# saamiya225/Graph-and-sequential-recommendation-systems

Measured on AMD Instinct MI355X. Metric: BPR training steps/sec (one step = K-layer LightGCN propagation + BPR loss + backward + Adam on a global batch of 2048 triplets), higher is better.
Workload: dtype bf16 (activation storage; f32 accumulation, parameters, gradients and Adam); 1 GPU; gowalla: 29858 users x 40981 items, 810128 train interactions, nnz(A_hat)=1620256, layers=3, dim=64, bpr_batch=2048; global_batch=2048, per_gpu_batch=2048, scaling_mode=strong, multi_gpu_status=n/a, parallelism=single GPU, act_dtype=bf16, xcd_remap=1, row_order=xcd

## Files before the change

graph-and-sequential-recommendation-systems_amd/_lib.py:

```python
import ctypes as C
import os

from . import build as _build

F32, BF16, FP8 = 0, 1, 2
ABI_VERSION = 13
MAX_LAYERS = 8

_c_i32p = C.POINTER(C.c_int32)
_c_i64p = C.POINTER(C.c_int64)
_c_f32p = C.POINTER(C.c_float)
_vp = C.c_void_p


def fp8_col_of_byte(d):
    import numpy as np
    b = np.arange(d)
    l, j, e = b // 16, (b % 16) // 4, b % 4
    return ((j * (d // 16) + l) * 4 + e).astype(np.int64)


class TrainConfig(C.Structure):
    _fields_ = [
        ("graph", _vp),
# ... 89 lines not shown
    "lgcn_train_step_cols_part2": (C.c_int, [_vp, _vp, _vp, _vp, C.c_int32, _vp, _vp]),
    "lgcn_dp_allreduce_sum_f32": (C.c_int, [_vp, _vp, C.c_int64, _vp]),
    "lgcn_dp_init_loopback": (C.c_int, [C.c_int, C.POINTER(_vp)]),
    "lgcn_dp_destroy": (None, [_vp]),
    "lgcn_dp_world": (C.c_int, [_vp]),
    "lgcn_dp_rank": (C.c_int, [_vp]),
    "lgcn_train_epoch_dp": (C.c_int, [_vp, _vp, _vp, _vp, _vp, C.c_int64, C.c_int32, C.c_int32, _vp, _vp, _vp, _vp]),
    "lgcn_rs_phase": (C.c_int, [_vp, C.c_int32, C.c_int32, _vp, _vp, _vp, C.c_int32, C.c_int32, C.c_int32, _vp, _vp, _vp]),
    "lgcn_rs_buffer": (C.c_int, [_vp, C.c_int32, C.c_int32, C.POINTER(_vp), C.POINTER(C.c_int32)]),
    "lgcn_ctx_set_dropout": (C.c_int, [_vp, C.c_float, C.c_uint64]),
    "lgcn_ctx_set_layer_weights": (C.c_int, [_vp, _vp, C.c_int32]),
    "lgcn_ctx_get_layer_weights": (C.c_int32, [_vp, _vp]),
    "lgcn_propagate_weighted": (C.c_int, [_vp, _vp, C.c_int, C.c_int, C.c_int, _vp, _vp, _vp, _vp]),
    "lgcn_dropout_mask": (C.c_int, [_vp, _vp, C.c_int64, C.c_int64, C.c_float, C.c_uint64, C.c_int64, _vp, _vp]),
    "lgcn_spmm_csr_drop": (C.c_int, [_vp, _vp, C.c_int, _vp, C.c_int, C.c_int, C.c_float, C.c_uint64, C.c_int64, C.c_int, _vp]),
    "lgcn_mf_create": (C.c_int, [C.POINTER(MfConfig), C.POINTER(_vp)]),
    "lgcn_mf_destroy": (None, [_vp]),
    "lgcn_mf_get_step": (C.c_int64, [_vp]),
    "lgcn_mf_set_step": (None, [_vp, C.c_int64]),
    "lgcn_mf_set_lr": (None, [_vp, C.c_double]),
    "lgcn_mf_train_step": (C.c_int, [_vp, _vp, _vp, _vp, C.c_int32, _vp, _vp]),
    "lgcn_mf_train_epoch": (C.c_int, [_vp, _vp, _vp, _vp, C.c_int64, C.c_int32, _vp, _vp]),
    "lgcn_mf_check": (C.c_int, [_vp, _vp]),
}

_LIB = None


class LgcnError(RuntimeError):
    pass


def load():
    global _LIB
    if _LIB is not None:
        return _LIB
    path = _build.LIB_PATH
    if os.environ.get("LGCN_LIB_PATH"):
        pass
    elif _build.is_stale():
        if _build.must_not_build():
            if not os.path.exists(path):
                raise LgcnError(
                    f"liblgcn_hip.so is missing at {path}; this process is a distributed rank or runs under a "
                    "profiler and will not compile it. Build it first (__graft_entry__.build()).")
        elif _build.find_hipcc() is not None:
# ... 380 lines not shown
```

graph-and-sequential-recommendation-systems_amd/csrc/lgcn_device.hip:

```cpp
#include <hip/hip_runtime.h>
#include <stdint.h>
#include <stdio.h>
#include <stdlib.h>
#include <string.h>
#include <math.h>
#include <algorithm>
#include <array>
#include <new>
#include <vector>

#include "lgcn_hip.h"
#include "lgcn_internal.h"

#define HIP_OK(expr)                                                            \
    do {                                                                        \
        hipError_t e_ = (expr);                                                 \
        if (e_ != hipSuccess) {                                                 \
            char buf_[256];                                                     \
            snprintf(buf_, sizeof buf_, "%s failed: %s", #expr, hipGetErrorString(e_)); \
            lgcn_set_error(buf_);                                               \
            return 10;                                                          \
        }                                                                       \
    } while (0)

// ... 848 lines not shown
    const float *X0; const void *Xl[LGCN_MAX_LAYERS + 1]; int K;
    int32_t n_users; int64_t N;
    const int32_t *users; const int32_t *pos; const int32_t *neg;
    int32_t B_local;
    int32_t shard;
    float inv_B;
    float lam;
    long long *G64;
    uint32_t *bitmap;
    uint32_t *stale_bitmap; int64_t bitmap_words;
    uint32_t *item_bitmap;
    float *contrib;
    int32_t exchange;
    const float *Xhub; int32_t hub_nnz;
    float *terms;
    int32_t terms_off, terms_stride;
    int32_t *err;
    int32_t dense_last;
    int32_t reg_ego;
    int32_t *cnt;
    int32_t cols_phase; float *erows; float *colsum;
    DropArgs dr;
    float w[LGCN_MAX_LAYERS + 1];
};

__device__ __forceinline__ float logsigmoid_f(float x) { return fminf(x, 0.f) - log1pf(expf(-fabsf(x))); }
__device__ __forceinline__ float sigmoid_neg_f(float x) {
    const float z = expf(-fabsf(x));
    return x < 0.f ? 1.f / (1.f + z) : z / (1.f + z);
}

__device__ __forceinline__ bool triplet_bad(const BprArgs &a, int b) {
    const int u = a.users[b], p = a.pos[b], n = a.neg[b];
    return u < 0 || u >= a.n_users || p < 0 || (int64_t)p + a.n_users >= a.N || n < 0 || (int64_t)n + a.n_users >= a.N;
}

template <int D>
__device__ __forceinline__ void triplet_finish(const BprArgs &a, int b, int l, const float *u, const float *p, const float *n,
                                               float ps, float ns, float rr);
template <int D>
__device__ __forceinline__ void triplet_loss_regs(const BprArgs &a, int b, int l, const float *u, const float *p, const float *n,
                                                  const float *u0 = nullptr, const float *p0 = nullptr, const float *n0 = nullptr) {
    constexpr int LPT = D < 64 ? D : 64, CPL = D / LPT;
    float ps = 0.f, ns = 0.f, ru = 0.f, rp = 0.f, rn = 0.f;
    const bool ego = a.reg_ego != 0;
    const float lam = ego ? 0.f : a.lam;
#pragma unroll
    for (int j = 0; j < CPL; j++) {
        ps += u[j] * p[j]; ns += u[j] * n[j];
        const float ur = ego ? u0[j] : u[j], pr = ego ? p0[j] : p[j], nr = ego ? n0[j] : n[j];
        ru += ur * ur; rp += pr * pr; rn += nr * nr;
    }
    float rr = ru + rp + rn;
#pragma unroll
    for (int off = 1; off < LPT; off <<= 1) {
        ps += __shfl_xor(ps, off); ns += __shfl_xor(ns, off); rr += __shfl_xor(rr, off);
    }
    if (a.cols_phase == 1) {
        const bool bad1 = triplet_bad(a, b);
        if (l == 0) { a.colsum[b] = bad1 ? 0.f : ps; a.colsum[a.B_local + b] = bad1 ? 0.f : ns; a.colsum[2 * a.B_local + b] = bad1 ? 0.f : rr; }
#pragma unroll
        for (int j = 0; j < CPL; j++) {
            a.erows[((int64_t)0 * a.B_local + b) * D + j * LPT + l] = u[j];
            a.erows[((int64_t)1 * a.B_local + b) * D + j * LPT + l] = p[j];
            a.erows[((int64_t)2 * a.B_local + b) * D + j * LPT + l] = n[j];
        }
        return;
    }
    triplet_finish<D>(a, b, l, u, p, n, ps, ns, rr);
}

template <int D>
__device__ __forceinline__ void triplet_finish(const BprArgs &a, int b, int l, const float *u, const float *p, const float *n,
                                               float ps, float ns, float rr) {
    constexpr int LPT = D < 64 ? D : 64, CPL = D / LPT;
    const float lam = a.reg_ego ? 0.f : a.lam;
    const bool tbad = triplet_bad(a, b);
    const float x = ps - ns;
    const float gb = tbad ? 0.f : -a.inv_B * sigmoid_neg_f(x);
    if (l == 0) {
        float *lt = a.exchange ? a.contrib + (int64_t)3 * a.shard * D : a.terms + a.terms_off;
        const int stride = a.exchange ? a.shard : a.terms_stride;
        lt[b] = tbad ? 0.f : logsigmoid_f(x);
        lt[stride + b] = tbad ? 0.f : rr;
    }
    if (tbad && !a.exchange) return;
    const int64_t rows[3] = {(int64_t)a.users[b], (int64_t)a.pos[b] + a.n_users, (int64_t)a.neg[b] + a.n_users};
#pragma unroll
    for (int c = 0; c < 3; c++) {
#pragma unroll
        for (int j = 0; j < CPL; j++) {
            float g = c == 0 ? gb * (p[j] - n[j]) + lam * u[j] : (c == 1 ? gb * u[j] + lam * p[j] : (-gb) * u[j] + lam * n[j]);
            if (a.G64 && !tbad)
                atomicAdd((unsigned long long *)(a.G64 + rows[c] * D + j * LPT + l),
                          (unsigned long long)__double2ll_rn((double)g * FIXED_SCALE));
            if (a.exchange) a.contrib[((int64_t)c * a.shard + b) * D + j * LPT + l] = tbad ? 0.f : g;
        }
        if (a.G64 && !tbad && l == 0) {
            atomicOr(a.bitmap + (rows[c] >> 5), 1u << (rows[c] & 31));
            if (a.cnt) atomicAdd(a.cnt + rows[c], 1);
            if (a.item_bitmap && c > 0) { const int64_t it = rows[c] - a.n_users; atomicOr(a.item_bitmap + (it >> 5), 1u << (it & 31)); }
        }
    }
}

#ifndef TRIPLET_HUB_NNZ
#define TRIPLET_HUB_NNZ 131072
#endif
#ifndef TRIPLET_HUB_CHUNK
#define TRIPLET_HUB_CHUNK 2048
#endif
#ifndef TRIPLET_MIN_WAVES
#define TRIPLET_MIN_WAVES 4
#endif
#ifndef TRIPLET_MIN_WAVES_F32
#define TRIPLET_MIN_WAVES_F32 7
#endif
#ifndef TRIPLET_U
#define TRIPLET_U LGCN_GATHER_U
#endif
#ifndef TRIPLET_WAVES
#define TRIPLET_WAVES 4
#endif
#ifndef TRIPLET_WAVES_BF16
#define TRIPLET_WAVES_BF16 3
#endif
// ... 469 lines not shown
    const int64_t blk = a.blk ? a.blk : (int64_t)3 * a.shard * D + 2 * a.shard;
    const float *src = a.gathered + r * blk + ((int64_t)c * a.shard + i) * D;
#pragma unroll
    for (int j = 0; j < CPT; j++)
        atomicAdd((unsigned long long *)(a.G64 + row * D + j * LPT + l),
                  (unsigned long long)__double2ll_rn((double)src[j * LPT + l] * FIXED_SCALE));
    if (l == 0) {
        atomicOr(a.bitmap + (row >> 5), 1u << (row & 31));
        if (a.cnt) atomicAdd(a.cnt + row, 1);
        if (a.item_bitmap && c > 0) { const int64_t it = row - a.n_users; atomicOr(a.item_bitmap + (it >> 5), 1u << (it & 31)); }
    }
}

template <int D>
__global__ void __launch_bounds__(256) k_g32(SlotArgs a) {
    constexpr int LPR = D / 4, SPB = 256 / LPR;
    const int s = blockIdx.x * SPB + threadIdx.x / LPR, l = threadIdx.x % LPR;
    if (s >= 3 * a.B) return;
    const int64_t row = slot_row(s / a.B, s % a.B, a.users, a.pos, a.neg, a.n_users, a.N);
    if (row < 0) return;
    store4(a.G32 + row * D + l * 4, loadv_fixed<4>(a.G64 + row * D + l * 4, a.div));
}

__global__ void __launch_bounds__(256) k_flag_rows(SlotArgs a) {
    const int s = blockIdx.x * 256 + threadIdx.x;
    if (s >= 3 * a.B) return;
    const int64_t row = slot_row(s / a.B, s % a.B, a.users, a.pos, a.neg, a.n_users, a.N);
    if (row >= 0) {
        atomicOr(a.bitmap + (row >> 5), 1u << (row & 31));
        if (a.cnt) atomicAdd(a.cnt + row, 1);
        if (a.item_bitmap && s >= a.B) { const int64_t it = row - a.n_users; atomicOr(a.item_bitmap + (it >> 5), 1u << (it & 31)); }
    }
}

template <int D>
__global__ void __launch_bounds__(256) k_finish(SlotArgs a) {
    constexpr int LPR = D / 4, SPB = 256 / LPR;
    const int s = blockIdx.x * SPB + threadIdx.x / LPR, l = threadIdx.x % LPR;
    if (s < 3 * a.B) {
        const int c = s / a.B, b = s % a.B;
        const int64_t row = slot_row(c, b, a.users, a.pos, a.neg, a.n_users, a.N);
        if (row >= 0) {
                    i64x2 *q = reinterpret_cast<i64x2 *>(a.G64 + row * D + l * 4);
            q[0] = i64x2{0, 0}; q[1] = i64x2{0, 0};
            if (l == 0) { a.bitmap[row >> 5] = 0u; if (a.cnt) a.cnt[row] = 0; }
        }
// ... 509 lines not shown
    int flip;
    void *act[LGCN_MAX_LAYERS + 1];
    int fwd_layers;
    float *g32;
    bf16_t *e0b;
    void *e0q;
    bool e0b_fresh;
    bool in_loop;
    lgcn_graph *hub_graph;
    int32_t hub_nnz;
    int64_t hub_rows;
    bool dp_local;
    int dp_rank;
    bool variant;
    float *tvar;
    uint32_t *item_bitmap;
    long long *gate_partials;
    long long *gate_total;
    int32_t gate_P, gate_wgs;
    int32_t *cnt;
    float *colsum;
    float drop_keep; uint64_t drop_seed; DropArgs dr;
    int32_t lw_n; float lw[LGCN_MAX_LAYERS + 1];
};
struct LoopScope {
    lgcn_ctx *x;
    explicit LoopScope(lgcn_ctx *x_) : x(x_) { x->in_loop = true; x->e0b_fresh = false; }
    ~LoopScope() { x->in_loop = false; x->e0b_fresh = false; }
};

extern "C" int lgcn_ctx_create(const lgcn_train_config *cfg, lgcn_ctx **out) {
    if (!cfg || !out) { lgcn_set_error("lgcn_ctx_create: null argument"); return 3; }
    const lgcn_train_config &c = *cfg;
    if (!c.graph || !c.E0 || !c.adam_m || !c.adam_v || !c.G64 ||
        !c.bitmap || !c.terms || !c.err) { lgcn_set_error("lgcn_ctx_create: null buffer"); return 3; }
    if (c.K < 1 || c.K > LGCN_MAX_LAYERS) { lgcn_set_error("lgcn_ctx_create: K out of range"); return 3; }
    if ((c.K > 1 || c.dense_last) && !c.act) { lgcn_set_error("lgcn_ctx_create: activation workspace missing"); return 3; }
    if (c.d != 32 && c.d != 64 && c.d != 128 && c.d != 256) { lgcn_set_error("embedding dim must be 32, 64, 128 or 256"); return 3; }
    if (check_dtype(c.act_dtype)) return 3;
    if (c.act_dtype == LGCN_FP8 && c.d < 64) { lgcn_set_error("lgcn_ctx_create: fp8 activation storage needs an embedding dim of 64, 128 or 256"); return 3; }
    if (c.act_dtype == LGCN_FP8 && (c.item_pop || c.i2i)) { lgcn_set_error("lgcn_ctx_create: fp8 activation storage is implemented for the default model, not with the optional branches"); return 3; }
    if (c.n_users <= 0 || c.n_users >= c.graph->n_rows || c.max_batch <= 0) { lgcn_set_error("lgcn_ctx_create: bad sizes"); return 3; }
    if (c.d > c.graph->d_max) { lgcn_set_error("lgcn_ctx_create: d exceeds the graph's d_max"); return 3; }
    const bool gate = c.item_pop != nullptr, smooth = c.i2i != nullptr;
    if (gate || smooth) {
        if (!c.dense_last) { lgcn_set_error("lgcn_ctx_create: the optional branches need dense_last = 1 (every layer propagated densely)"); return 3; }
        const int64_t m_items = c.graph->n_rows - c.n_users;
        if (smooth && (!c.i2i_t || c.i2i->n_rows != m_items || c.i2i_t->n_rows != m_items || c.i2i->d_max < c.d || c.i2i_t->d_max < c.d)) {
            lgcn_set_error("lgcn_ctx_create: i2i / i2i_t must be [m_items, m_items] graphs with d_max >= d"); return 3; }
        if (gate && (!c.gate_params || !c.gate_adam_m || !c.gate_adam_v || !c.gate_grad || c.pop_hidden < 1 || c.pop_hidden > GATE_HMAX ||
                     c.gate_hidden < 1 || c.gate_hidden > GATE_HMAX || c.d > 128 || !(c.pop_gate_temp > 0.f))) {
            lgcn_set_error("lgcn_ctx_create: popularity gate needs its parameter / Adam buffers, hidden sizes in 1..64, d <= 128, temperature > 0"); return 3; }
    }
    if (c.reg_ego && (gate || smooth)) { lgcn_set_error("lgcn_ctx_create: reg_ego (upstream's L2 term) is defined for the default model only, not with the optional branches"); return 3; }
    lgcn_ctx *x = new (std::nothrow) lgcn_ctx;
    if (!x) { lgcn_set_error("out of memory"); return 4; }
    x->c = c; x->step = 0; x->N = c.graph->n_rows; x->cnt = nullptr; x->colsum = nullptr;
    x->drop_keep = 1.f; x->drop_seed = 0; x->dr = DropArgs{};
    x->lw_n = 0; for (int k = 0; k <= LGCN_MAX_LAYERS; k++) x->lw[k] = 0.f;
    x->bm_words = (x->N + 31) / 32; x->flip = 0;
    const size_t stride = table_bytes(x->N, c.d, c.act_dtype);
    for (int k = 0; k <= LGCN_MAX_LAYERS; k++) x->act[k] = nullptr;
    x->fwd_layers = c.dense_last ? c.K : c.K - 1;
    for (int k = 1; k <= x->fwd_layers; k++) x->act[k] = (char *)c.act + (size_t)(k - 1) * stride;
    x->g32 = nullptr; x->e0b = nullptr; x->e0q = nullptr; x->e0b_fresh = false; x->in_loop = false; x->dp_local = false; x->dp_rank = -1;
    x->hub_graph = nullptr; x->hub_nnz = 0; x->hub_rows = 0;
    x->variant = gate || smooth; x->tvar = nullptr; x->item_bitmap = nullptr; x->gate_partials = nullptr; x->gate_total = nullptr; x->gate_P = 0; x->gate_wgs = 0;
    const size_t gbytes = (size_t)x->N * c.d * sizeof(float);
    bool ok = hipMalloc((void **)&x->g32, gbytes) == hipSuccess && hipMemset(x->g32, 0, gbytes) == hipSuccess;
    if (ok) ok = hipMalloc((void **)&x->colsum, sizeof(float) * 3 * (size_t)c.max_batch) == hipSuccess;
    if (ok && c.reg_ego) ok = hipMalloc((void **)&x->cnt, sizeof(int32_t) * (size_t)x->N) == hipSuccess && hipMemset(x->cnt, 0, sizeof(int32_t) * (size_t)x->N) == hipSuccess;
    if (ok && x->variant) ok = hipMalloc((void **)&x->tvar, gbytes) == hipSuccess;
    if (ok && smooth) {
        const size_t wb = sizeof(uint32_t) * (size_t)((x->N - c.n_users + 31) / 32);
        ok = hipMalloc((void **)&x->item_bitmap, wb) == hipSuccess && hipMemset(x->item_bitmap, 0, wb) == hipSuccess;
    }
    if (ok && gate) {
        x->gate_P = 2 * c.pop_hidden + c.d * c.pop_hidden + c.d + 2 * c.d * c.gate_hidden + 2 * c.gate_hidden + 1;
        x->gate_wgs = (c.max_batch + GATE_TPB - 1) / GATE_TPB;
        ok = hipMalloc((void **)&x->gate_partials, sizeof(long long) * ((size_t)x->gate_wgs + 1) * x->gate_P) == hipSuccess;
        if (ok) x->gate_total = x->gate_partials + (size_t)x->gate_wgs * x->gate_P;
    }
// ... 1 lines not shown
    if (ok && c.act_dtype == LGCN_FP8 && c.K >= 2) ok = hipMalloc(&x->e0q, table_bytes(x->N, c.d, LGCN_FP8)) == hipSuccess;
    if (ok && !c.dense_last) {
        const int32_t thr = c.hub_nnz == 0 ? TRIPLET_HUB_NNZ : c.hub_nnz;
        if (thr > 0) {
            std::vector<int32_t> ip((size_t)x->N + 1), hubs;
            ok = hipMemcpy(ip.data(), c.graph->indptr, sizeof(int32_t) * ip.size(), hipMemcpyDeviceToHost) == hipSuccess;
            for (int64_t r = 0; ok && r < x->N; r++) if (ip[(size_t)r + 1] - ip[(size_t)r] > thr) hubs.push_back((int32_t)r);
            if (ok && !hubs.empty()) {
                int32_t *dh = nullptr;
                ok = hipMalloc((void **)&dh, sizeof(int32_t) * hubs.size()) == hipSuccess &&
                     hipMemcpy(dh, hubs.data(), sizeof(int32_t) * hubs.size(), hipMemcpyHostToDevice) == hipSuccess;
                const int32_t hub_chunk = c.hub_chunk > 0 ? c.hub_chunk : TRIPLET_HUB_CHUNK;
                if (ok) ok = graph_create_impl(c.graph->indptr, c.graph->indices, c.graph->vals, x->N, c.graph->nnz, c.d, dh,
                                               (int64_t)hubs.size(), nullptr, hub_chunk, &x->hub_graph) == 0;
                if (dh) (void)hipFree(dh);
                x->hub_nnz = thr; x->hub_rows = (int64_t)hubs.size();
            }
        }
    }
    if (!ok) {
        if (x->g32) (void)hipFree(x->g32);
        if (x->colsum) (void)hipFree(x->colsum);
        if (x->cnt) (void)hipFree(x->cnt);
        if (x->tvar) (void)hipFree(x->tvar);
        if (x->item_bitmap) (void)hipFree(x->item_bitmap);
        if (x->gate_partials) (void)hipFree(x->gate_partials);
        if (x->e0b) (void)hipFree(x->e0b);
        if (x->e0q) (void)hipFree(x->e0q);
        if (x->hub_graph) lgcn_graph_destroy(x->hub_graph);
        delete x;
        lgcn_set_error("lgcn_ctx_create: cannot allocate the library-owned tables (N*d*4 bytes fp32 gradient rows, N*d*2 bf16 parameters)");
        return 4;
    }
    *out = x;
    return 0;
}
extern "C" void lgcn_ctx_destroy(lgcn_ctx *ctx) {
    if (!ctx) return;
    if (ctx->g32) (void)hipFree(ctx->g32);
    if (ctx->colsum) (void)hipFree(ctx->colsum);
    if (ctx->cnt) (void)hipFree(ctx->cnt);
    if (ctx->tvar) (void)hipFree(ctx->tvar);
    if (ctx->item_bitmap) (void)hipFree(ctx->item_bitmap);
    if (ctx->gate_partials) (void)hipFree(ctx->gate_partials);
    if (ctx->e0b) (void)hipFree(ctx->e0b);
    if (ctx->e0q) (void)hipFree(ctx->e0q);
    if (ctx->hub_graph) lgcn_graph_destroy(ctx->hub_graph);
    delete ctx;
}
extern "C" int lgcn_ctx_set_dp_local(lgcn_ctx *ctx, int on) {
    if (!ctx) { lgcn_set_error("lgcn_ctx_set_dp_local: null context"); return 3; }
    ctx->dp_local = on != 0; ctx->dp_rank = -1;
    return 0;
}
extern "C" int64_t lgcn_ctx_get_step(const lgcn_ctx *ctx) { return ctx ? ctx->step : -1; }
extern "C" int64_t lgcn_ctx_hub_rows(const lgcn_ctx *ctx) { return (ctx && ctx->hub_graph) ? ctx->hub_rows : 0; }
extern "C" void lgcn_ctx_set_step(lgcn_ctx *ctx, int64_t s) { if (ctx) ctx->step = s; }
extern "C" void lgcn_ctx_set_lr(lgcn_ctx *ctx, double lr) { if (ctx) ctx->c.lr = lr; }
extern "C" int lgcn_ctx_set_dropout(lgcn_ctx *ctx, float keep_prob, uint64_t seed) {
    if (!ctx) { lgcn_set_error("lgcn_ctx_set_dropout: null context"); return 3; }
    if (!drop_prob_ok(keep_prob)) { lgcn_set_error("lgcn_ctx_set_dropout: dropout keep_prob must be in (0, 1]"); return 3; }
    if (ctx->c.act_dtype == LGCN_FP8) { lgcn_set_error("lgcn_ctx_set_dropout: edge dropout is not implemented for LGCN_FP8 activation storage"); return 3; }
    if (ctx->variant) { lgcn_set_error("lgcn_ctx_set_dropout: edge dropout is not implemented with the optional branches (item-item smoothing / popularity gate)"); return 3; }
    if (ctx->lw_n && keep_prob < 1.f) { lgcn_set_error("lgcn_ctx_set_dropout: edge dropout is not implemented together with layer weights (lgcn_ctx_set_layer_weights)"); return 3; }
    ctx->drop_keep = keep_prob; ctx->drop_seed = seed; ctx->dr = DropArgs{};
    return 0;
}
static int refuse_dropout(const lgcn_ctx *x, const char *who) {
    if (!x || !(x->drop_keep < 1.f)) return 0;
    char buf[192];
    snprintf(buf, sizeof buf, "%s: edge dropout (lgcn_ctx_set_dropout) is implemented for the single-GPU step only", who);
    lgcn_set_error(buf);
    return 3;
}

// ... 56 lines not shown
}

static int run_bpr(lgcn_ctx *x, const int32_t *users, const int32_t *pos, const int32_t *neg,
                   int32_t B_global, int32_t b_off, int32_t B_local, int32_t shard, bool atomics, bool exchange, hipStream_t st,
                   bool count_slots = true, int cols_phase = 0) {
    const lgcn_train_config &c = x->c;
    BprArgs a{};
    a.reg_ego = c.reg_ego; a.cnt = (atomics && count_slots) ? x->cnt : nullptr;
    a.dr = x->dr;
    const bool wts = x->lw_n != 0;
    for (int k = 0; k < x->lw_n; k++) a.w[k] = x->lw[k];
    a.cols_phase = cols_phase; a.erows = c.contrib; a.colsum = x->colsum;
    a.indptr = c.graph->indptr; a.indices = c.graph->indices; a.vals = c.graph->vals; a.X0 = c.E0; a.K = c.K;
    for (int k = 1; k <= x->fwd_layers; k++) a.Xl[k] = x->act[k];
    a.dense_last = c.dense_last;
    a.n_users = c.n_users; a.N = x->N;
    a.users = users + b_off; a.pos = pos + b_off; a.neg = neg + b_off;
    a.B_local = B_local; a.shard = shard;
    a.inv_B = 1.0f / (float)B_global; a.lam = c.decay / (float)B_global;
    a.G64 = atomics ? (long long *)c.G64 : nullptr; a.bitmap = c.bitmap + x->flip * x->bm_words;
    a.stale_bitmap = c.bitmap + (x->flip ^ 1) * x->bm_words; a.bitmap_words = x->bm_words;
    a.contrib = c.contrib; a.terms = c.terms; a.err = c.err; a.exchange = exchange ? 1 : 0;
    a.terms_off = exchange ? 0 : b_off; a.terms_stride = B_global;
    if (cols_phase == 2) {
        if (B_local <= 0) return 0;
        DISPATCH_D(c.d, {
            const int tpb = 256 / (D < 64 ? D : 64);
            hipLaunchKernelGGL((k_cols_finish<D>), dim3((unsigned)((B_local + tpb - 1) / tpb)), dim3(256), 0, st, a);
        });
        return 0;
    }
    if (x->hub_graph && !c.dense_last && B_local > 0) {
        { int rc0 = graph_acquire(x->hub_graph, st); if (rc0) return rc0; }
        SpmmArgs h = graph_spmm(x->hub_graph);
        h.X = c.K == 1 ? (const void *)c.E0 : x->act[c.K - 1]; h.Y = x->g32; h.remap = c.xcd_remap; h.dr = x->dr;
        int rc = launch_spmm<0>(h, c.d, c.K == 1 ? LGCN_F32 : c.act_dtype, LGCN_F32, st);
        if (rc) return rc;
        a.Xhub = x->g32; a.hub_nnz = x->hub_nnz;
    }
    if (B_local <= 0) {
        HIP_OK(hipMemsetAsync(a.stale_bitmap, 0, sizeof(uint32_t) * (size_t)x->bm_words, st));
        return 0;
    }
    DISPATCH_D(c.d, {
        if (c.act_dtype == LGCN_FP8) {
            if constexpr (D >= 64) {
// ... 128 lines not shown
    s.blk = gathered ? dp_block_floats(x, shard) : 0;
    s.item_bitmap = (x->variant && c.i2i) ? x->item_bitmap : nullptr;
    s.cnt = x->cnt;
    return s;
}
static unsigned scatter_grid(const lgcn_ctx *x, int32_t B) {
    const int spb = 256 / (x->c.d < 64 ? x->c.d : 64);
    return (unsigned)((3 * (int64_t)B + spb - 1) / spb);
}
static unsigned slot_grid(const lgcn_ctx *x, int32_t B) {
    const int spb = 256 / (x->c.d / 4);
    return (unsigned)((3 * (int64_t)B + spb - 1) / spb);
}

static void *bwd_buffer(const lgcn_ctx *x, int k) {
    return (x->c.K == 2) ? x->act[1] : x->act[1 + ((x->c.K - k) & 1)];
}

static int backward_layer(lgcn_ctx *x, int k, const int32_t *users, const int32_t *pos, const int32_t *neg, int32_t B,
                          const float *gathered, int32_t shard, float *loss_out, bool fused_finish, hipStream_t st) {
    const lgcn_train_config &c = x->c;
    const bool first = (k == c.K), last = (k == 1);
    if (first) {
        SlotArgs s = slot_args(x, users, pos, neg, B, gathered, shard, 1, loss_out);
        DISPATCH_D(c.d, hipLaunchKernelGGL((k_g32<D>), dim3(slot_grid(x, B)), dim3(256), 0, st, s));
        if (x->variant && c.i2i) {
            { int rc0 = graph_acquire(c.i2i_t, st); if (rc0) return rc0; }
            const int64_t ioff = (int64_t)c.n_users * c.d, m_items = x->N - c.n_users;
            SpmmArgs h = graph_spmm(c.i2i_t);
            h.G32 = x->g32 + ioff; h.bitmap = x->item_bitmap; h.Y = x->tvar + ioff; h.div = (float)(c.K + 1); h.remap = c.xcd_remap;
            int rc = launch_spmm<M_SPARSE | M_ADDG>(h, c.d, LGCN_F32, LGCN_F32, st);
            if (rc) return rc;
            HIP_OK(hipMemcpyAsync(x->g32 + ioff, x->tvar + ioff, sizeof(float) * (size_t)m_items * c.d, hipMemcpyDeviceToDevice, st));
            const int64_t words = (x->N + 31) / 32;
            hipLaunchKernelGGL(k_flag_range, dim3((unsigned)((words + 255) / 256 < 64 ? (words + 255) / 256 : 64)), dim3(256), 0, st,
                               c.bitmap + x->flip * x->bm_words, (int64_t)c.n_users, x->N);
        }
    }
    SpmmArgs a = base_spmm(x);
    a.dr = x->dr; a.dr.tr = 1;
    a.X = first ? nullptr : bwd_buffer(x, k + 1);
    if (!last) a.Y = bwd_buffer(x, k);
    else {
        const double bc1 = 1.0 - pow(c.beta1, (double)x->step);
        const double bc2 = 1.0 - pow(c.beta2, (double)x->step);
        a.P = c.E0; a.M = c.adam_m; a.V = c.adam_v;
        a.cnt = x->cnt; a.lam = c.decay / (float)B;
        a.Pb = (x->e0b && x->in_loop && fused_finish) ? x->e0b : nullptr;
// ... 65 lines not shown
}

extern "C" int lgcn_train_step(lgcn_ctx *x, const int32_t *users, const int32_t *pos, const int32_t *neg,
                               int32_t B, float *loss_out, void *stream) {
    int rc = check_batch(x, users, pos, neg, B);
    if (rc) return rc;
    if (!loss_out) { lgcn_set_error("train step: loss_out is null"); return 3; }
    hipStream_t st = (hipStream_t)stream;
    x->dr = make_drop(x->drop_keep, x->drop_seed, x->step, 0);
    if ((rc = run_forward(x, st))) return rc;
    if (x->variant) rc = run_variant_loss(x, users, pos, neg, B, 0, B, B, true, false, st);
    else rc = run_bpr(x, users, pos, neg, B, 0, B, B, true, false, st);
    if (rc) return rc;
    if ((rc = run_backward(x, users, pos, neg, B, nullptr, B, 1, loss_out, st))) return rc;
    HIP_OK(hipGetLastError());
    return 0;
}

extern "C" int lgcn_train_epoch(lgcn_ctx *x, const int32_t *users, const int32_t *pos, const int32_t *neg,
                                int64_t T, int32_t B, float *loss_out, void *stream) {
    if (T <= 0) return 0;
    if (!x) { lgcn_set_error("train epoch: null context"); return 3; }
    LoopScope scope(x);
    int64_t i = 0;
    for (int64_t t = 0; t < T; t += B, i++) {
        const int32_t b = (int32_t)((T - t) < B ? (T - t) : B);
        int rc = lgcn_train_step(x, users + t, pos + t, neg + t, b, loss_out + 3 * i, stream);
        if (rc) return rc;
    }
    return 0;
}

extern "C" int lgcn_train_step_dp_part1(lgcn_ctx *x, const int32_t *users, const int32_t *pos, const int32_t *neg,
                                        int32_t B_global, int32_t world, int32_t rank, void *stream) {
    int rc = check_batch(x, users, pos, neg, B_global);
    if (rc) return rc;
    if ((rc = refuse_dropout(x, "lgcn_train_step_dp_part1"))) return rc;
    if ((rc = refuse_layer_weights(x, "lgcn_train_step_dp_part1"))) return rc;
    if (!x->c.contrib) { lgcn_set_error("dp step: cfg.contrib exchange buffer missing"); return 3; }
    if (world < 1 || rank < 0 || rank >= world) { lgcn_set_error("dp step: bad world/rank"); return 3; }
    const int32_t shard = (B_global + world - 1) / world;
    const int32_t b_off = rank * shard;
    int32_t B_local = B_global - b_off;
    if (B_local > shard) B_local = shard;
    if (B_local < 0) B_local = 0;
    hipStream_t st = (hipStream_t)stream;
    if ((rc = run_forward(x, st))) return rc;
    if (x->variant) rc = run_variant_loss(x, users, pos, neg, B_global, b_off, B_local, shard, x->dp_local, true, st);
    else rc = run_bpr(x, users, pos, neg, B_global, b_off, B_local, shard, x->dp_local, true, st);
    if (rc) return rc;
    x->dp_rank = rank;
// ... 262 lines not shown
```

graph-and-sequential-recommendation-systems_amd/model.py:

```python
import ctypes as C

import numpy as np
import torch
from torch import nn
import torch.nn.functional as F

from . import world
from . import _lib


def _act_code(name):
    return {'fp32': _lib.F32, 'bf16': _lib.BF16, 'fp8': _lib.FP8}[name]


def _act_tables(n_tables, N, d, act_dtype, dev):
    if act_dtype == _lib.FP8:
        return torch.zeros(n_tables, int(_lib.load().lgcn_table_bytes(N, d, _lib.FP8)), dtype=torch.uint8, device=dev)
    return torch.zeros(n_tables, N, d, dtype=torch.float32 if act_dtype == _lib.F32 else torch.bfloat16, device=dev)


def _check_layer_weights(w, K, what):
    w = np.asarray(w, dtype=np.float64).reshape(-1)
    if w.size != K + 1:
        raise ValueError(f"{what}: {w.size} layer weights for --layer {K} (K + 1 = {K + 1} are needed)")
# ... 377 lines not shown
                    st[key] = torch.zeros(P, dtype=torch.float32, device=dev)
            st['item_pop'] = self.item_pop_scalar.to(device=dev, dtype=torch.float32).contiguous()
            cfg.item_pop, cfg.gate_params = st['item_pop'].data_ptr(), self._gate_flat.data_ptr()
            cfg.gate_adam_m, cfg.gate_adam_v, cfg.gate_grad = st['gate_m'].data_ptr(), st['gate_v'].data_ptr(), st['gate_grad'].data_ptr()
            cfg.pop_hidden, cfg.gate_hidden = self.pop_hidden, self.gate_hidden
            cfg.gate_entropy_coeff, cfg.pop_gate_temp = self.gate_entropy_coeff, self.pop_gate_temp
        st['dense_last'] = dense_last
        h = C.c_void_p()
        _lib.check(lib.lgcn_ctx_create(C.byref(cfg), C.byref(h)), "lgcn_ctx_create")
        lib.lgcn_ctx_set_step(h, old_step)
        if self.dropout:
            rc = lib.lgcn_ctx_set_dropout(h, self.keep_prob, int(self.config.get('seed', 2020)) & (2 ** 64 - 1))
            if rc:
                msg = lib.lgcn_last_error()
                lib.lgcn_ctx_destroy(h)
                raise _lib.LgcnError(f"lgcn_ctx_set_dropout failed (rc={rc}): {msg.decode() if msg else ''}")
        if self.layer_weights is not None:
            w = np.ascontiguousarray(self.layer_weights, dtype=np.float32)
            rc = lib.lgcn_ctx_set_layer_weights(h, w.ctypes.data_as(C.c_void_p), int(w.size))
            if rc:
                msg = lib.lgcn_last_error()
                lib.lgcn_ctx_destroy(h)
                raise _lib.LgcnError(f"lgcn_ctx_set_layer_weights failed (rc={rc}): {msg.decode() if msg else ''}")
        st['ctx'], st['max_batch'], st['dp_world'], st['table_ptr'] = h, max_batch, dp_world, self._table.data_ptr()
        st['ctx_rows'] = rows

    def _dense_last(self, batch):
        mode = str(self.config.get('dense_last', 'auto'))
        if mode in ('0', '1'):
            return mode == '1'
        deg = np.diff(self._adj.indptr).astype(np.float64)
        du, di = deg[:self.n_users], deg[self.n_users:]
        per_triplet = du.mean() + (di * di).sum() / max(di.sum(), 1.0) + di.mean()
        return bool(batch * per_triplet > 0.3 * self._adj.nnz)

    def _spmm(self, x):
        return self._state()['graph'].spmm(x.float(), _lib.F32)

    @property
    def i2i_active(self):
        return self.use_item_item and self._i2i is not None and self.i2i_alpha > 0.0

    @property
    def has_variants(self):
        return self.use_pop_gate or self.i2i_active

# ... 380 lines not shown
```

include/lgcn_hip.h:

```cpp
#ifndef LGCN_HIP_H
#define LGCN_HIP_H

#include <stdint.h>

#ifdef __cplusplus
extern "C" {
#endif

#define LGCN_ABI_VERSION 13
#define LGCN_MAX_LAYERS 8

enum { LGCN_F32 = 0, LGCN_BF16 = 1, LGCN_FP8 = 2 };
int64_t lgcn_table_bytes(int64_t n_rows, int32_t d, int32_t dtype);
int lgcn_to_fp8(const float *src, void *dst, int64_t n_rows, int32_t d, void *stream);

int lgcn_abi_version(void);
const char *lgcn_last_error(void);
int lgcn_device_available(void);

void lgcn_sampling_seed(unsigned int seed);
int lgcn_sampling_randint(int end);
int lgcn_sample_negative(int user_num, int item_num, int64_t train_num,
                         const int64_t *indptr, const int32_t *indices,
                         int neg_num, int32_t *S_out);
// ... 82 lines not shown
    float pop_gate_temp;
    int32_t reg_ego;
} lgcn_train_config;

int lgcn_ctx_create(const lgcn_train_config *cfg, lgcn_ctx **out);
void lgcn_ctx_destroy(lgcn_ctx *ctx);
int64_t lgcn_ctx_get_step(const lgcn_ctx *ctx);
int64_t lgcn_ctx_hub_rows(const lgcn_ctx *ctx);
void lgcn_ctx_set_step(lgcn_ctx *ctx, int64_t step);
void lgcn_ctx_set_lr(lgcn_ctx *ctx, double lr);
int lgcn_ctx_set_dropout(lgcn_ctx *ctx, float keep_prob, uint64_t seed);
int lgcn_ctx_set_layer_weights(lgcn_ctx *ctx, const float *w_host, int32_t n);
int32_t lgcn_ctx_get_layer_weights(const lgcn_ctx *ctx, float *w_out);
int lgcn_ctx_set_dp_local(lgcn_ctx *ctx, int on);

int lgcn_train_step(lgcn_ctx *ctx, const int32_t *users, const int32_t *pos, const int32_t *neg,
                    int32_t B, float *loss_out, void *stream);

int lgcn_train_step_i64(lgcn_ctx *ctx, const int64_t *users, const int64_t *pos, const int64_t *neg,
                        int32_t B, int32_t *ids_scratch, float *loss_out, void *stream);

int lgcn_train_epoch(lgcn_ctx *ctx, const int32_t *users, const int32_t *pos, const int32_t *neg,
                     int64_t T, int32_t B, float *loss_out, void *stream);

int64_t lgcn_dp_block_floats(const lgcn_ctx *ctx, int32_t B_global, int32_t world);
int lgcn_train_step_dp_part1(lgcn_ctx *ctx, const int32_t *users, const int32_t *pos,
                             const int32_t *neg, int32_t B_global, int32_t world, int32_t rank,
                             void *stream);
int lgcn_train_step_dp_dense_part1(lgcn_ctx *ctx, const int32_t *users, const int32_t *pos,
                                   const int32_t *neg, int32_t B_global, int32_t world, int32_t rank,
                                   void *stream);
int lgcn_ctx_gate_total(const lgcn_ctx *ctx, void **buf, int32_t *count);
int lgcn_train_step_dp_part2(lgcn_ctx *ctx, const int32_t *users, const int32_t *pos,
                             const int32_t *neg, int32_t B_global, int32_t world,
                             const float *gathered, float *loss_out, void *stream);

int lgcn_train_step_cols_part1(lgcn_ctx *ctx, const int32_t *users, const int32_t *pos, const int32_t *neg,
                               int32_t B, float **partials, void *stream);
int lgcn_train_step_cols_part2(lgcn_ctx *ctx, const int32_t *users, const int32_t *pos, const int32_t *neg,
                               int32_t B, float *loss_out, void *stream);

int lgcn_eval_topk(const float *E, int32_t n_users, int32_t m_items, int32_t d,
                   const int32_t *users, int32_t n_eval,
                   const int64_t *train_indptr, const int32_t *train_indices,
                   int32_t K, int32_t *topk_items, float *topk_scores, void *stream);
int64_t lgcn_eval_mask_words(int32_t m_items, int32_t n_eval);
// ... 100 lines not shown
```

Baseline: 8517 steps/s.

## Fold G64-to-G32 conversion into BPR triplet kernel using per-row multiplicity tickets

Before the epoch's steps run, a per-segment kernel computes how many times each gradient row occurs within each batch, using an LDS hash. The BPR finish kernel then writes rows that occur once straight to G32. Rows that occur several times use a per-row arrival ticket so the last contributor converts the fixed-point G64 sum into G32. This removes the separate k_g32 conversion launch and most 64-bit atomics. The cost is a multiplicity pre-pass, a ticket array, vmcnt waits and acquire fences inside the loss kernel.

```diff
diff --git a/graph-and-sequential-recommendation-systems_amd/_lib.py b/graph-and-sequential-recommendation-systems_amd/_lib.py
--- a/graph-and-sequential-recommendation-systems_amd/_lib.py
+++ b/graph-and-sequential-recommendation-systems_amd/_lib.py
@@ -135,6 +135,10 @@
     "lgcn_mf_train_step": (C.c_int, [_vp, _vp, _vp, _vp, C.c_int32, _vp, _vp]),
     "lgcn_mf_train_epoch": (C.c_int, [_vp, _vp, _vp, _vp, C.c_int64, C.c_int32, _vp, _vp]),
     "lgcn_mf_check": (C.c_int, [_vp, _vp]),
+    "lgcn_ctx_set_fold_g32": (C.c_int, [_vp, C.c_int]),
+    "lgcn_ctx_folded_steps": (C.c_int64, [_vp]),
+    "lgcn_ctx_copy_arrivals": (C.c_int, [_vp, _vp, C.c_int64]),
+    "lgcn_slot_multiplicity": (C.c_int, [_vp, _vp, _vp, C.c_int64, C.c_int32, C.c_int32, C.c_int64, _vp, _vp]),
 }
 
 _LIB = None
diff --git a/graph-and-sequential-recommendation-systems_amd/csrc/lgcn_device.hip b/graph-and-sequential-recommendation-systems_amd/csrc/lgcn_device.hip
--- a/graph-and-sequential-recommendation-systems_amd/csrc/lgcn_device.hip
+++ b/graph-and-sequential-recommendation-systems_amd/csrc/lgcn_device.hip
@@ -894,6 +894,7 @@
     int32_t cols_phase; float *erows; float *colsum;
     DropArgs dr;
     float w[LGCN_MAX_LAYERS + 1];
+    const uint16_t *mult; float *G32; float gdiv; int32_t *arrive;
 };
 
 __device__ __forceinline__ float logsigmoid_f(float x) { return fminf(x, 0.f) - log1pf(expf(-fabsf(x))); }
@@ -940,6 +941,39 @@
         return;
     }
     triplet_finish<D>(a, b, l, u, p, n, ps, ns, rr);
+}
+
+#ifndef FOLD_TICKET_ALL
+#define FOLD_TICKET_ALL 0
+#endif
+template <int D>
+__device__ __forceinline__ void fold_close_rows(const BprArgs &a, const int64_t (&rows)[3], const int (&m)[3], int l) {
+    constexpr int LPT = D < 64 ? D : 64, CPL = D / LPT, MIN_SHARED = FOLD_TICKET_ALL ? 1 : 2;
+    typedef __attribute__((address_space(1))) unsigned long long gu64;
+    if (m[0] < MIN_SHARED && m[1] < MIN_SHARED && m[2] < MIN_SHARED) return;
+    asm volatile("s_waitcnt vmcnt(0)" ::: "memory");
+    const int ml = l == 0 ? m[0] : (l == 1 ? m[1] : m[2]);
+    const int64_t rl = l == 0 ? rows[0] : (l == 1 ? rows[1] : rows[2]);
+    int ticket = -1;
+    if (l < 3 && ml >= MIN_SHARED) ticket = __hip_atomic_fetch_add(a.arrive + rl, 1, __ATOMIC_RELAXED, __HIP_MEMORY_SCOPE_AGENT);
+    bool last[3];
+#pragma unroll
+    for (int c = 0; c < 3; c++) {
+        const int t = LPT == 64 ? __builtin_amdgcn_readlane(ticket, c) : __shfl(ticket, c, LPT);
+        last[c] = m[c] >= MIN_SHARED && t == m[c] - 1;
+    }
+    if (!(last[0] || last[1] || last[2])) return;
+    __builtin_amdgcn_fence(__ATOMIC_ACQUIRE, "agent");
+    if (l < 3 && ml >= MIN_SHARED && ticket == ml - 1) __hip_atomic_store(a.arrive + rl, 0, __ATOMIC_RELAXED, __HIP_MEMORY_SCOPE_AGENT);
+#pragma unroll
+    for (int c = 0; c < 3; c++) {
+        if (!last[c]) continue;
+#pragma unroll
+        for (int j = 0; j < CPL; j++) {
+            const long long q = (long long)__hip_atomic_load((gu64 *)(a.G64 + rows[c] * D + j * LPT + l), __ATOMIC_RELAXED, __HIP_MEMORY_SCOPE_AGENT);
+            a.G32[rows[c] * D + j * LPT + l] = (float)((double)q * FIXED_INV) / a.gdiv;
+        }
+    }
 }
 
 template <int D>
@@ -958,14 +992,23 @@
     }
     if (tbad && !a.exchange) return;
     const int64_t rows[3] = {(int64_t)a.users[b], (int64_t)a.pos[b] + a.n_users, (int64_t)a.neg[b] + a.n_users};
+    int mm[3] = {0, 0, 0};
+    if (a.mult) {
+#pragma unroll
+        for (int c = 0; c < 3; c++) mm[c] = (int)a.mult[c * a.B_local + b];
+    }
 #pragma unroll
     for (int c = 0; c < 3; c++) {
+        const int m = mm[c];
+        const bool direct = !FOLD_TICKET_ALL && m == 1;
 #pragma unroll
         for (int j = 0; j < CPL; j++) {
             float g = c == 0 ? gb * (p[j] - n[j]) + lam * u[j] : (c == 1 ? gb * u[j] + lam * p[j] : (-gb) * u[j] + lam * n[j]);
-            if (a.G64 && !tbad)
-                atomicAdd((unsigned long long *)(a.G64 + rows[c] * D + j * LPT + l),
-                          (unsigned long long)__double2ll_rn((double)g * FIXED_SCALE));
+            if (a.G64 && !tbad) {
+                const long long q = __double2ll_rn((double)g * FIXED_SCALE);
+                if (direct) a.G32[rows[c] * D + j * LPT + l] = (float)((double)q * FIXED_INV) / a.gdiv;
+                else atomicAdd((unsigned long long *)(a.G64 + rows[c] * D + j * LPT + l), (unsigned long long)q);
+            }
             if (a.exchange) a.contrib[((int64_t)c * a.shard + b) * D + j * LPT + l] = tbad ? 0.f : g;
         }
         if (a.G64 && !tbad && l == 0) {
@@ -974,6 +1017,7 @@
             if (a.item_bitmap && c > 0) { const int64_t it = rows[c] - a.n_users; atomicOr(a.item_bitmap + (it >> 5), 1u << (it & 31)); }
         }
     }
+    if (a.G64 && !tbad && a.mult) fold_close_rows<D>(a, rows, mm, l);
 }
 
 #ifndef TRIPLET_HUB_NNZ
@@ -1489,6 +1533,96 @@
     store4(a.G32 + row * D + l * 4, loadv_fixed<4>(a.G64 + row * D + l * 4, a.div));
 }
 
+#define SLOT_MULT_HMAX 16384
+#define SLOT_MULT_THREADS 1024
+struct SlotMultArgs {
+    const int32_t *users; const int32_t *pos; const int32_t *neg;
+    int64_t T; int32_t B; int32_t n_users; int64_t N;
+    uint16_t *out; int32_t H;
+};
+__global__ void __launch_bounds__(SLOT_MULT_THREADS) k_slot_mult(SlotMultArgs a) {
+    extern __shared__ int32_t slot_mult_lds[];
+    int32_t *keys = slot_mult_lds, *cnts = slot_mult_lds + a.H;
+    const int64_t t0 = (int64_t)blockIdx.x * a.B;
+    const int bn = (int)((a.T - t0) < a.B ? (a.T - t0) : a.B);
+    const int32_t *users = a.users + t0, *pos = a.pos + t0, *neg = a.neg + t0;
+    const uint32_t mask = (uint32_t)a.H - 1u;
+    for (int i = threadIdx.x; i < a.H; i += SLOT_MULT_THREADS) { keys[i] = -1; cnts[i] = 0; }
+    __syncthreads();
+#pragma unroll 1
+    for (int b = threadIdx.x; b < bn; b += SLOT_MULT_THREADS) {
+        const int32_t r0 = (int32_t)slot_row(0, b, users, pos, neg, a.n_users, a.N);
+        if (r0 < 0) continue;
+        const int32_t r1 = pos[b] + a.n_users, r2 = neg[b] + a.n_users;
+#pragma unroll 1
+        for (int c = 0; c < 3; c++) {
+            const int32_t row = c == 0 ? r0 : (c == 1 ? r1 : r2);
+            uint32_t h = drop_fmix32((uint32_t)row) & mask;
+            for (int probe = 0; probe < a.H; probe++, h = (h + 1u) & mask) {
+                const int32_t old = atomicCAS(&keys[h], -1, row);
+                if (old == -1 || old == row) { atomicAdd(&cnts[h], 1); break; }
+            }
+        }
+    }
+    __syncthreads();
+#pragma unroll 1
+    for (int b = threadIdx.x; b < bn; b += SLOT_MULT_THREADS) {
+        const int32_t r0 = (int32_t)slot_row(0, b, users, pos, neg, a.n_users, a.N);
+        const int32_t r1 = pos[b] + a.n_users, r2 = neg[b] + a.n_users;
+#pragma unroll 1
+        for (int c = 0; c < 3; c++) {
+            const int32_t row = c == 0 ? r0 : (c == 1 ? r1 : r2);
+            int m = 0;
+            if (r0 >= 0) {
+                uint32_t h = drop_fmix32((uint32_t)row) & mask;
+                for (int probe = 0; probe < a.H; probe++, h = (h + 1u) & mask)
+                    if (keys[h] == row) { m = cnts[h]; break; }
+            }
+            a.out[3 * t0 + (int64_t)c * bn + b] = (uint16_t)m;
+        }
+    }
+}
+static int32_t slot_mult_hash(int32_t B) {
+    if (B <= 0) return 0;
+    int64_t H = 64;
+    while (3 * H < 12 * (int64_t)B) H <<= 1;
+    return H <= SLOT_MULT_HMAX ? (int32_t)H : 0;
+}
+static int64_t fold_segment_steps() {
+    const char *e = getenv("LGCN_FOLD_SEGMENT");
+    const long v = e ? atol(e) : 0;
+    return v > 0 ? (int64_t)v : 1024;
+}
+static int launch_slot_mult(const int32_t *users, const int32_t *pos, const int32_t *neg, int64_t T, int32_t B, int32_t n_users,
+                            int64_t N, uint16_t *out, hipStream_t st) {
+    SlotMultArgs a{};
+    a.users = users; a.pos = pos; a.neg = neg; a.T = T; a.B = B; a.n_users = n_users; a.N = N; a.out = out; a.H = slot_mult_hash(B);
+    const size_t lds = sizeof(int32_t) * 2 * (size_t)a.H;
+    static bool attr_set[64] = {};
+    int dev = 0;
+    HIP_OK(hipGetDevice(&dev));
+    if (dev < 0 || dev >= 64 || !attr_set[dev]) {
+        HIP_OK(hipFuncSetAttribute((const void *)k_slot_mult, hipFuncAttributeMaxDynamicSharedMemorySize, (int)(sizeof(int32_t) * 2 * SLOT_MULT_HMAX)));
+        if (dev >= 0 && dev < 64) attr_set[dev] = true;
+    }
+    hipLaunchKernelGGL(k_slot_mult, dim3((unsigned)((T + B - 1) / B)), dim3(SLOT_MULT_THREADS), lds, st, a);
+    return 0;
+}
+extern "C" int lgcn_slot_multiplicity(const int32_t *users, const int32_t *pos, const int32_t *neg, int64_t T, int32_t B,
+                                      int32_t n_users, int64_t N, uint16_t *mult_out, void *stream) {
+    if (T <= 0) return 0;
+    if (!users || !pos || !neg || !mult_out) { lgcn_set_error("lgcn_slot_multiplicity: null argument"); return 3; }
+    if (B <= 0 || n_users <= 0 || N <= n_users || N > 0x7fffffffLL) { lgcn_set_error("lgcn_slot_multiplicity: bad sizes (0 < B, 0 < n_users < N < 2^31)"); return 3; }
+    if (!slot_mult_hash(B)) { lgcn_set_error("lgcn_slot_multiplicity: the row ids of a batch of B triplets do not fit the LDS hash (B <= 4096)"); return 3; }
+    const int64_t seg = fold_segment_steps() * B;
+    for (int64_t t = 0; t < T; t += seg) {
+        int rc = launch_slot_mult(users + t, pos + t, neg + t, (T - t) < seg ? (T - t) : seg, B, n_users, N, mult_out + 3 * t, (hipStream_t)stream);
+        if (rc) return rc;
+    }
+    HIP_OK(hipGetLastError());
+    return 0;
+}
+
 __global__ void __launch_bounds__(256) k_flag_rows(SlotArgs a) {
     const int s = blockIdx.x * 256 + threadIdx.x;
     if (s >= 3 * a.B) return;
@@ -2044,6 +2178,11 @@
     float *colsum;
     float drop_keep; uint64_t drop_seed; DropArgs dr;
     int32_t lw_n; float lw[LGCN_MAX_LAYERS + 1];
+    bool fold_g32;
+    uint16_t *mult; int64_t mult_cap;
+    const uint16_t *fold_mult;
+    int32_t *arrive;
+    int64_t folded_steps;
 };
 struct LoopScope {
     lgcn_ctx *x;
@@ -2080,6 +2219,7 @@
     x->c = c; x->step = 0; x->N = c.graph->n_rows; x->cnt = nullptr; x->colsum = nullptr;
     x->drop_keep = 1.f; x->drop_seed = 0; x->dr = DropArgs{};
     x->lw_n = 0; for (int k = 0; k <= LGCN_MAX_LAYERS; k++) x->lw[k] = 0.f;
+    x->fold_g32 = true; x->mult = nullptr; x->mult_cap = 0; x->fold_mult = nullptr; x->arrive = nullptr; x->folded_steps = 0;
     x->bm_words = (x->N + 31) / 32; x->flip = 0;
     const size_t stride = table_bytes(x->N, c.d, c.act_dtype);
     for (int k = 0; k <= LGCN_MAX_LAYERS; k++) x->act[k] = nullptr;
@@ -2127,6 +2267,7 @@
         if (x->g32) (void)hipFree(x->g32);
         if (x->colsum) (void)hipFree(x->colsum);
         if (x->cnt) (void)hipFree(x->cnt);
+        if (x->arrive) (void)hipFree(x->arrive);
         if (x->tvar) (void)hipFree(x->tvar);
         if (x->item_bitmap) (void)hipFree(x->item_bitmap);
         if (x->gate_partials) (void)hipFree(x->gate_partials);
@@ -2145,6 +2286,8 @@
     if (ctx->g32) (void)hipFree(ctx->g32);
     if (ctx->colsum) (void)hipFree(ctx->colsum);
     if (ctx->cnt) (void)hipFree(ctx->cnt);
+    if (ctx->arrive) (void)hipFree(ctx->arrive);
+    if (ctx->mult) (void)hipFree(ctx->mult);
     if (ctx->tvar) (void)hipFree(ctx->tvar);
     if (ctx->item_bitmap) (void)hipFree(ctx->item_bitmap);
     if (ctx->gate_partials) (void)hipFree(ctx->gate_partials);
@@ -2156,6 +2299,20 @@
 extern "C" int lgcn_ctx_set_dp_local(lgcn_ctx *ctx, int on) {
     if (!ctx) { lgcn_set_error("lgcn_ctx_set_dp_local: null context"); return 3; }
     ctx->dp_local = on != 0; ctx->dp_rank = -1;
+    return 0;
+}
+extern "C" int lgcn_ctx_set_fold_g32(lgcn_ctx *ctx, int on) {
+    if (!ctx) { lgcn_set_error("lgcn_ctx_set_fold_g32: null context"); return 3; }
+    ctx->fold_g32 = on != 0;
+    return 0;
+}
+extern "C" int64_t lgcn_ctx_folded_steps(const lgcn_ctx *ctx) { return ctx ? ctx->folded_steps : -1; }
+extern "C" int lgcn_ctx_copy_arrivals(const lgcn_ctx *ctx, int32_t *dst_host, int64_t n) {
+    if (!ctx || !dst_host) { lgcn_set_error("lgcn_ctx_copy_arrivals: null argument"); return 3; }
+    if (ctx->variant || n < 0 || n > ctx->N) { lgcn_set_error("lgcn_ctx_copy_arrivals: the context has no arrival array of that size"); return 3; }
+    if (!ctx->arrive) { memset(dst_host, 0, sizeof(int32_t) * (size_t)n); return 0; }
+    HIP_OK(hipDeviceSynchronize());
+    HIP_OK(hipMemcpy(dst_host, ctx->arrive, sizeof(int32_t) * (size_t)n, hipMemcpyDeviceToHost));
     return 0;
 }
 extern "C" int64_t lgcn_ctx_get_step(const lgcn_ctx *ctx) { return ctx ? ctx->step : -1; }
@@ -2258,6 +2415,9 @@
     a.stale_bitmap = c.bitmap + (x->flip ^ 1) * x->bm_words; a.bitmap_words = x->bm_words;
     a.contrib = c.contrib; a.terms = c.terms; a.err = c.err; a.exchange = exchange ? 1 : 0;
     a.terms_off = exchange ? 0 : b_off; a.terms_stride = B_global;
+    if (x->fold_mult && atomics && !exchange && cols_phase == 0 && b_off == 0 && B_local == B_global) {
+        a.mult = x->fold_mult; a.G32 = x->g32; a.gdiv = x->lw_n ? 1.f : (float)(c.K + 1); a.arrive = x->arrive;
+    }
     if (cols_phase == 2) {
         if (B_local <= 0) return 0;
         DISPATCH_D(c.d, {
@@ -2432,8 +2592,10 @@
     const lgcn_train_config &c = x->c;
     const bool first = (k == c.K), last = (k == 1);
     if (first) {
-        SlotArgs s = slot_args(x, users, pos, neg, B, gathered, shard, 1, loss_out);
-        DISPATCH_D(c.d, hipLaunchKernelGGL((k_g32<D>), dim3(slot_grid(x, B)), dim3(256), 0, st, s));
+        if (!x->fold_mult) {
+            SlotArgs s = slot_args(x, users, pos, neg, B, gathered, shard, 1, loss_out);
+            DISPATCH_D(c.d, hipLaunchKernelGGL((k_g32<D>), dim3(slot_grid(x, B)), dim3(256), 0, st, s));
+        }
         if (x->variant && c.i2i) {
             { int rc0 = graph_acquire(c.i2i_t, st); if (rc0) return rc0; }
             const int64_t ioff = (int64_t)c.n_users * c.d, m_items = x->N - c.n_users;
@@ -2545,11 +2707,39 @@
     if (T <= 0) return 0;
     if (!x) { lgcn_set_error("train epoch: null context"); return 3; }
     LoopScope scope(x);
-    int64_t i = 0;
+    const bool fold = x->fold_g32 && !x->variant && !x->hub_graph && users && pos && neg &&
+                      B > 0 && B <= x->c.max_batch && x->N <= 0x7fffffffLL && slot_mult_hash(B) != 0;
+    const int64_t seg = fold_segment_steps();
+    if (fold) {
+        if (!x->arrive) {
+            HIP_OK(hipMalloc((void **)&x->arrive, sizeof(int32_t) * (size_t)x->N));
+            HIP_OK(hipMemsetAsync(x->arrive, 0, sizeof(int32_t) * (size_t)x->N, (hipStream_t)stream));
+        }
+        const int64_t bmax = x->c.max_batch < 4096 ? x->c.max_batch : 4096;
+        const int64_t need = 3 * (B > bmax ? (int64_t)B : bmax) * seg;
+        if (x->mult_cap < need) {
+            if (x->mult) (void)hipFree(x->mult);
+            x->mult = nullptr; x->mult_cap = 0;
+            HIP_OK(hipMalloc((void **)&x->mult, sizeof(uint16_t) * (size_t)need));
+            x->mult_cap = need;
+        }
+    }
+    int64_t i = 0, seg_t0 = 0;
     for (int64_t t = 0; t < T; t += B, i++) {
         const int32_t b = (int32_t)((T - t) < B ? (T - t) : B);
+        if (fold) {
+            if (i % seg == 0) {
+                seg_t0 = t;
+                const int64_t Ts = (T - t) < seg * B ? (T - t) : seg * B;
+                int rc = launch_slot_mult(users + t, pos + t, neg + t, Ts, B, x->c.n_users, x->N, x->mult, (hipStream_t)stream);
+                if (rc) return rc;
+            }
+            x->fold_mult = x->mult + 3 * (t - seg_t0);
+        }
         int rc = lgcn_train_step(x, users + t, pos + t, neg + t, b, loss_out + 3 * i, stream);
+        x->fold_mult = nullptr;
         if (rc) return rc;
+        if (fold) x->folded_steps += 1;
     }
     return 0;
 }
diff --git a/graph-and-sequential-recommendation-systems_amd/model.py b/graph-and-sequential-recommendation-systems_amd/model.py
--- a/graph-and-sequential-recommendation-systems_amd/model.py
+++ b/graph-and-sequential-recommendation-systems_amd/model.py
@@ -423,6 +423,12 @@
                 msg = lib.lgcn_last_error()
                 lib.lgcn_ctx_destroy(h)
                 raise _lib.LgcnError(f"lgcn_ctx_set_layer_weights failed (rc={rc}): {msg.decode() if msg else ''}")
+        if str(self.config.get('fold_g32', 1)).strip().lower() in ('0', 'false', 'off'):
+            rc = lib.lgcn_ctx_set_fold_g32(h, 0)
+            if rc:
+                msg = lib.lgcn_last_error()
+                lib.lgcn_ctx_destroy(h)
+                raise _lib.LgcnError(f"lgcn_ctx_set_fold_g32 failed (rc={rc}): {msg.decode() if msg else ''}")
         st['ctx'], st['max_batch'], st['dp_world'], st['table_ptr'] = h, max_batch, dp_world, self._table.data_ptr()
         st['ctx_rows'] = rows
 
diff --git a/include/lgcn_hip.h b/include/lgcn_hip.h
--- a/include/lgcn_hip.h
+++ b/include/lgcn_hip.h
@@ -128,6 +128,12 @@
 
 int lgcn_train_epoch(lgcn_ctx *ctx, const int32_t *users, const int32_t *pos, const int32_t *neg,
                      int64_t T, int32_t B, float *loss_out, void *stream);
+
+int lgcn_ctx_set_fold_g32(lgcn_ctx *ctx, int on);
+int64_t lgcn_ctx_folded_steps(const lgcn_ctx *ctx);
+int lgcn_ctx_copy_arrivals(const lgcn_ctx *ctx, int32_t *dst_host, int64_t n);
+int lgcn_slot_multiplicity(const int32_t *users, const int32_t *pos, const int32_t *neg, int64_t T, int32_t B,
+                           int32_t n_users, int64_t N, uint16_t *mult_out, void *stream);
 
 int64_t lgcn_dp_block_floats(const lgcn_ctx *ctx, int32_t B_global, int32_t world);
 int lgcn_train_step_dp_part1(lgcn_ctx *ctx, const int32_t *users, const int32_t *pos,
```

After: 8696 steps/s (median of 6 runs). 1.02x the previous value.
